# SandraLouise/SVJedi-graph

Hardware: NVIDIA B200
Metric: gaf_alignments_filtered_assigned_per_sec (higher is better)
Workload: dtype u8/int64

## Files before the change

### include/svjg.h

```cpp
#ifndef SVJG_H
#define SVJG_H

#include <stddef.h>
#include <stdint.h>

#ifdef __cplusplus
extern "C" {
#endif

#define SVJG_OK 0
#define SVJG_E_CUDA 1
#define SVJG_E_ARG 2
#define SVJG_E_IO 3
#define SVJG_E_JSON 4
#define SVJG_E_INPUT 5
#define SVJG_E_HITS_OVERFLOW 6
#define SVJG_E_NOMEM 7
#define SVJG_E_UNSUPPORTED 8

#define SVJG_BAD_COLUMNS 1
#define SVJG_BAD_INT 2
#define SVJG_BAD_ALEN 3
#define SVJG_BAD_PATH 4
#define SVJG_BAD_ALTNODE 5
// ... 18 lines not shown
int64_t svjg_tables_alt_node_len(const svjg_tables *t, const char *name, uint32_t len);
uint64_t svjg_tables_image_hash(const svjg_tables *t);
const char *svjg_tables_sv_id(const svjg_tables *t, uint32_t i, uint32_t *len);
uint32_t svjg_tables_find_sv(const svjg_tables *t, const char *sv_id, uint32_t len);
#define SVJG_FLAG_EXACT_CHECKS 1u
#define SVJG_FLAG_FORCE_GENERAL 2u
int svjg_tables_set_flags(svjg_tables *t, uint32_t flags);
int svjg_tables_clone(const svjg_tables *t, svjg_tables **out);
int svjg_tables_to_device(svjg_tables *t, int device);

typedef struct svjg_filter_stats {
    uint64_t n_hits;
    uint64_t n_records;
    uint64_t n_multi;
    uint64_t n_checks;
    uint64_t status;
    uint64_t err_offset;
    uint64_t n_generic;
    uint64_t n_exact;
} svjg_filter_stats;

int svjg_filter_reset(uint32_t *d_counts, uint32_t num_sv, svjg_filter_stats *d_stats, void *stream);
int svjg_filter_device(const svjg_tables *t, const uint8_t *d_gaf, uint64_t n_bytes, uint64_t base_offset,
                       int64_t d_over, uint32_t *d_counts, uint32_t *d_hit_sv2, uint32_t *d_hit_off,
                       uint32_t *d_hit_len, uint64_t hit_cap, svjg_filter_stats *d_stats, void *stream);

uint64_t svjg_translate_newlines(uint8_t *p, uint64_t n);

#define SVJG_TUNE_TILE_BYTES 1
#define SVJG_TUNE_TILE_LINES 2
#define SVJG_TUNE_SCAN_BLOCKS 3
#define SVJG_TUNE_SCAN_ONLY 4
#define SVJG_TUNE_POOL_UNITS 5
int svjg_filter_tune(int knob, int value);
int svjg_filter_profile(int enable);
int svjg_filter_scan_ms(float *ms);

int svjg_filter_host(svjg_tables *t, const uint8_t *gaf, uint64_t n_bytes, int64_t d_over, uint32_t *counts,
                     uint32_t *hit_sv2, uint64_t *hit_off, uint32_t *hit_len, uint64_t hit_cap,
                     svjg_filter_stats *stats);

int svjg_filter_json_host(svjg_tables *t, const uint8_t *gaf, uint64_t n_bytes, int64_t d_over, uint32_t *counts,
                          svjg_filter_stats *stats, const char **json, uint64_t *json_len);
int svjg_filter_json_begin(svjg_tables *t, const uint8_t *gaf, uint64_t n_bytes, int64_t d_over, uint32_t *counts,
                           svjg_filter_stats *stats);
int svjg_filter_json_finish(svjg_tables *t, const char **json, uint64_t *json_len);
int svjg_filter_json_begin_at(svjg_tables *t, const uint8_t *gaf, uint64_t n_bytes, uint64_t base, int64_t d_over,
                              uint32_t *counts, svjg_filter_stats *stats);
int svjg_filter_json_gather(svjg_tables **ts, int n, const uint32_t *counts_sum);
int svjg_filter_json_write(svjg_tables *t, const char *path, uint64_t slice_bytes, uint64_t *json_len);

int svjg_hits_min_identity(const uint8_t *gaf, uint64_t n_bytes, uint32_t *hit_sv2, uint64_t *hit_off, uint32_t *hit_len,
                           uint64_t *n_hits, double min_identity, uint32_t *counts, uint32_t num_sv);

#define SVJG_GT_GENOTYPED 1
#define SVJG_GT_HALVED_0 2
#define SVJG_GT_HALVED_1 4
#define SVJG_GT_NEED_K 8

int svjg_genotype_device(const uint32_t *d_counts, const uint32_t *d_sv_index, const uint8_t *d_svtype,
                         uint32_t n, int64_t min_support, double log10_1me, double log10_e,
                         double log10_half, const double *d_lut, uint32_t lut_nmax,
                         const double *d_k_override, int64_t *d_pl, uint8_t *d_gt, uint32_t *d_ad2,
                         uint8_t *d_flags, void *stream);

int svjg_genotype_host(const uint32_t *counts, uint32_t num_counts, const uint32_t *sv_index, const uint8_t *svtype,
// ... 84 lines not shown
```

### svjedi-graph_b200/csrc/filter.cu

```cuda
#include <cooperative_groups.h>
#include <cuda_runtime.h>

#include <algorithm>
#include <cstdlib>
#include <map>
#include <mutex>

#include "svjg_internal.h"

namespace cg = cooperative_groups;
using namespace svjg;

namespace {

constexpr int TILE_MIN = 1024;
constexpr int TILE_LINES = 30;
constexpr int LOOKAHEAD = 1024;
constexpr int HEAD = 32;
constexpr int WARPS = 4;
constexpr int THREADS = WARPS * 32;
constexpr int SPARE = 32;

template <int MB_, int TILE_MAX_>
struct Geo {
    static constexpr int MB = MB_;
    static constexpr int TILE_MAX = TILE_MAX_;
    static constexpr int WIN = HEAD + TILE_MAX + LOOKAHEAD;
    static constexpr int NLCAP = WIN / 20 + 1;
    static constexpr int BMWORDS = WIN / 32 + 3;
    static constexpr int OFF_NL = WIN + SPARE;
    static constexpr int OFF_TAB = (OFF_NL + 2 * NLCAP + 15) & ~15;
    static constexpr int OFF_XD = OFF_TAB + 4 * BMWORDS;
    static constexpr int OFF_NS = OFF_XD + 4 * BMWORDS;
    static constexpr int OFF_TKO = OFF_NS + 4 * BMWORDS;
    static constexpr int OFF_LREC = (OFF_TKO + 32 + 15) & ~15;
    static constexpr int WARP_SMEM = (OFF_LREC + 32 * 8 + 127) & ~127;
    static constexpr int SMEM = WARP_SMEM * WARPS;
    static_assert(TILE_MAX % 32 == 0 && WIN + SPARE < 65536, "window offsets are 16 bit");
    static_assert((SMEM + 1024 + 64) * MB <= 233472, "MB blocks must fit an SM's 228 KB of shared memory");
};
typedef Geo<6, 4992> Geo6;
typedef Geo<8, 3360> Geo8;

constexpr int FLAT_THREADS = 256;

constexpr uint32_t FLAG_EXACT_CHECKS = SVJG_FLAG_EXACT_CHECKS;
constexpr uint32_t FLAG_FORCE_GENERAL = SVJG_FLAG_FORCE_GENERAL;
constexpr uint32_t FLAG_STOP_AFTER_SCAN = 1u << 8;
constexpr uint32_t COMMA_PATH = 0xFFFFFFFFu;

struct Scratch {
    uint32_t *cnt;
    uint32_t *exact;
    uint4 *slab;
    uint4 *pool;
    uint32_t cap_exact, cap_pool;
};

struct FilterArgs {
    const uint8_t *gaf;
    uint64_t n;
    uint64_t base;
    int64_t d_over;
    DevTables tb;
    uint32_t *counts;
    uint32_t *hit_sv2, *hit_off, *hit_len;
    uint64_t *hit_off64;
    uint64_t hit_cap;
    unsigned long long *stats;
    uint32_t flags;
    uint32_t one;
    Scratch sc;
    uint32_t skip;
    uint32_t tile_max;
    uint32_t tile_lines;
};

struct Local {
    uint32_t n_rec = 0, n_multi = 0, n_generic = 0;
    uint64_t n_checks = 0;
};
// ... 614 lines not shown
    }
    return v;
}

__device__ __forceinline__ uint64_t warp_incl_scan64(uint64_t v, int lane) {
#pragma unroll
    for (int d = 1; d < 32; d <<= 1) {
        uint64_t o = __shfl_up_sync(0xFFFFFFFFu, v, d);
        if (lane >= d) v += o;
    }
    return v;
}

__device__ __forceinline__ uint32_t bm_bits(const uint32_t *bm, uint32_t pos) {
    const uint32_t w = pos >> 5;
    return __funnelshift_r(bm[w], bm[w + 1], pos & 31u);
}
__device__ __forceinline__ uint32_t low_bits(int n) { return __funnelshift_lc(0xFFFFFFFFu, 0u, uint32_t(max(n, 0))); }
__device__ __forceinline__ uint32_t next_tab(const uint32_t *bm, uint32_t pos, uint32_t end) {
    for (uint32_t q = pos; q < end; q += 32) {
        const uint32_t m = bm_bits(bm, q) & low_bits(int(end - q));
        if (m) return q + uint32_t(__ffs(m) - 1);
    }
    return end;
}
__device__ __forceinline__ uint64_t bm64(const uint32_t *bm, uint32_t pos) {
    const uint32_t w = pos >> 5, sh = pos & 31u;
    const uint32_t b0 = bm[w], b1 = bm[w + 1], b2 = bm[w + 2];
    return (uint64_t(__funnelshift_r(b1, b2, sh)) << 32) | __funnelshift_r(b0, b1, sh);
}
__device__ __forceinline__ uint64_t low_bits64(int n) { return (uint64_t(low_bits(n - 32)) << 32) | low_bits(n); }

__device__ __forceinline__ uint32_t dec4(uint32_t w) {
    uint32_t t = w & 0x0F0F0F0Fu;
    t = t * 10u + (t >> 8);
    t &= 0x00FF00FFu;
    return (t * 100u + (t >> 16)) & 0xFFFFu;
}
__device__ __forceinline__ uint32_t clear_low_bytes(uint32_t w, int n) {
    return w & __funnelshift_lc(0u, 0xFFFFFFFFu, uint32_t(max(n, 0)) * 8u);
}
__device__ __forceinline__ bool pnode_find(const DevTables &tb, uint64_t c0, uint64_t c1, uint32_t ka, uint32_t kb,
                                           uint32_t &id, uint32_t &alt_len, uint32_t &roles) {
    uint32_t i = pnode_hash(c0, c1, ka, kb) & tb.pnode_mask;
    for (;;) {
        const uint4 *sp = reinterpret_cast<const uint4 *>(tb.pnodes + i);
        const uint4 lo = __ldg(sp), hi = __ldg(sp + 1);
        if (!hi.z) return false;
        if (lo.x == uint32_t(c0) && lo.y == uint32_t(c0 >> 32) && lo.z == uint32_t(c1) && lo.w == uint32_t(c1 >> 32) &&
            hi.x == ka && hi.y == kb) {
            id = (hi.z & PN_ID_MASK) - 1u;
            roles = hi.z >> 28;
            alt_len = hi.w;
            return true;
        }
        i = (i + 1) & tb.pnode_mask;
    }
}

__device__ __forceinline__ uint32_t link_dirs(uint32_t rolesA, uint32_t sA, uint32_t rolesB, uint32_t sB) {
    const uint32_t fwd = (rolesA >> sA) & (rolesB >> (2u + sB)) & 1u;
    const uint32_t rev = (rolesB >> (sB ^ 1u)) & (rolesA >> (2u + (sA ^ 1u))) & 1u;
    return fwd | (rev << 1);
}

struct SmemBytes {
    const uint8_t *p;
    __device__ __forceinline__ uint32_t u8(uint32_t i) const { return p[i]; }
    __device__ __forceinline__ uint32_t u32(uint32_t al) const { return *reinterpret_cast<const uint32_t *>(p + al); }
};
// ... 168 lines not shown
        bad |= __any_sync(0xFFFFFFFFu, act && !n.plain);
        total += __shfl_sync(0xFFFFFFFFu, warp_incl_scan64(n.nlen, lane), 31);
        from = __shfl_sync(0xFFFFFFFFu, nxt, 31);
    }
    __syncwarp();
    if (bad) return false;
    bool clash = false;
    for (uint32_t c0 = 0; c0 < cnt; c0 += 32) {
        const uint32_t t = c0 + uint32_t(lane);
        const uint32_t mine = t < cnt ? __ldcg(&slab[t].z) : 0u;
        const uint32_t upto = min(c0 + 32u, cnt);
        for (uint32_t j = 0; j < upto; ++j) clash |= j < t && t < cnt && __ldcg(&slab[j].z) == mine;
    }
    if (__any_sync(0xFFFFFFFFu, clash)) return false;
    uint64_t before = 0;
    for (uint32_t c0 = 0; c0 < cnt; c0 += 32) {
        const uint32_t t = c0 + uint32_t(lane);
        const bool act = t < cnt;
        const uint4 me = act ? __ldcg(slab + t) : make_uint4(NO_NODE, 0, 0, 0);
        const uint4 lf = act && t ? __ldcg(slab + t - 1) : make_uint4(NO_NODE, 0, 0, 0);
        const uint64_t incl = warp_incl_scan64(me.y, lane);
        const uint64_t pre = before + incl - me.y;
        const bool ok = (int64_t(pre) - lts >= a.d_over) && (int64_t(total - pre) - ltail >= a.d_over);
        const uint32_t dirs = link_dirs(lf.w >> 1, lf.w & 1u, me.w >> 1, me.w & 1u);
        const bool want = act && t && lf.x != NO_NODE && me.x != NO_NODE && dirs && (ok || (a.flags & FLAG_EXACT_CHECKS));
        probe_links(a, want, lf.x, lf.w & 1u, me.x, me.w & 1u, dirs, ok, off, len, lt_mask, n_checks);
        before += __shfl_sync(0xFFFFFFFFu, incl, 31);
    }
    n_checks = __reduce_add_sync(0xFFFFFFFFu, n_checks);
    if (lane == 0 && n_checks) atomicAdd(a.stats + 3, (unsigned long long)n_checks);
    return true;
}

template <class G>
__global__ void __launch_bounds__(THREADS, G::MB) scan_kernel(const __grid_constant__ FilterArgs a) {
    extern __shared__ __align__(128) uint8_t smem_all[];
    __shared__ __align__(8) uint64_t mbars[WARPS];
    __shared__ uint32_t next_tile[WARPS];

    const int lane = threadIdx.x & 31, warp = threadIdx.x >> 5;
    const uint32_t lt_mask = (1u << lane) - 1u;
    uint8_t *win = smem_all + warp * G::WARP_SMEM;
    uint16_t *nl = reinterpret_cast<uint16_t *>(win + G::OFF_NL);
    uint32_t *tabb = reinterpret_cast<uint32_t *>(win + G::OFF_TAB);
    uint32_t *xdb = reinterpret_cast<uint32_t *>(win + G::OFF_XD);
    uint32_t *nsb = reinterpret_cast<uint32_t *>(win + G::OFF_NS);
    uint8_t *tko = win + G::OFF_TKO;
    uint2 *lrec = reinterpret_cast<uint2 *>(win + G::OFF_LREC);
    uint64_t *mbar = &mbars[warp];
    const SmemBytes src{win};

    if (lane == 0) mbar_init(mbar, 1);
    for (int i = lane; i < G::BMWORDS; i += 32) tabb[i] = 0, xdb[i] = 0, nsb[i] = 0;
    for (int i = G::WIN + lane; i < G::WIN + SPARE; i += 32) win[i] = 0;
    __syncwarp();
    uint32_t phase = 0;
    uint32_t u_rec = 0, u_multi = 0, n_checks = 0;
    const uint32_t one = a.one;
    const uint32_t n_workers = gridDim.x * WARPS;

    cudaGridDependencySynchronize();
    cudaTriggerProgrammaticLaunchCompletion();
    const uint32_t tile_bytes = a.sc.cnt[4];
    const uint32_t n_tiles = uint32_t((a.n + tile_bytes - 1) / tile_bytes);
    const uint32_t win_bytes = HEAD + tile_bytes + LOOKAHEAD, n_pairs = win_bytes / 32u;

    for (uint32_t tile = blockIdx.x * WARPS + warp; tile < n_tiles; tile = next_tile[warp], __syncwarp()) {
        const uint64_t tile_start = uint64_t(tile) * tile_bytes;
        const uint64_t g0 = tile_start ? tile_start - HEAD : 0;
        const uint32_t dst0 = tile_start ? 0 : HEAD;
        uint64_t g1 = tile_start + tile_bytes + LOOKAHEAD;
        if (g1 > a.n) g1 = a.n;
        const bool at_eof = (g1 == a.n);
        const uint32_t nbytes = uint32_t(g1 - g0);
        const uint32_t bulk = nbytes & ~15u;
        const uint32_t valid_end = dst0 + nbytes;
        const uint32_t wbase = uint32_t(tile_start) - HEAD;

        if (lane == 0) {
            if (bulk) {
                asm volatile("fence.proxy.async.shared::cta;" ::: "memory");
// ... 113 lines not shown
                    }
                    plain &= pe < e && pe > ps;
                    const uint32_t n7 = min(pe + 1u, e);
                    uint64_t tt = bm64(tabb, n7);
                    const uint64_t xt = bm64(xdb, n7) & ~tt;
                    plain &= xt != 0;
                    const uint32_t l7 = uint32_t(__ffsll((long long)xt)) - 1u;
                    tt &= low_bits64(int(l7));
                    const uint32_t ntab = uint32_t(__popcll(tt));
                    const bool last_is_tab = l7 != 0 && ((tt >> ((l7 - 1u) & 63u)) & 1ull) != 0;
                    plain &= (ntab == 6 && last_is_tab) || (ntab == 5 && !last_is_tab && n7 + l7 == e);
                    plain &= (tt & ((tt >> 1) | 1ull)) == 0;
                    c6 = pe;
                    c7 = n7 + uint32_t(__ffsll((long long)tt)) - 1u;
                    tt &= tt - 1;
                    c8 = n7 + uint32_t(__ffsll((long long)tt)) - 1u;
                    tt &= tt - 1;
                    c9 = n7 + uint32_t(__ffsll((long long)tt)) - 1u;
                    tt &= tt - 1;
                    const uint32_t p10 = n7 + uint32_t(__ffsll((long long)tt)) - 1u;
                    plain = plain && win[p10 + 1] != '0';
                    if (!plain) {
                        exact = true;
                    } else if (!is_delim(win[ps])) {
                        exact = has_comma(win, ps, pe);
                    } else if (ntok >= 2) {
                        if (a.flags & FLAG_FORCE_GENERAL) exact = true;
                        else want = ntok;
                    }
                }
            }
            __syncwarp();
            int32_t ts = 0, tail = 0;
            if (want) {
                const uint32_t n_tlen = c7 - c6 - 1u, n_ts = c8 - c7 - 1u, n_te = c9 - c8 - 1u;
                if (max(n_tlen, max(n_ts, n_te)) <= 9u) {
                    ts = int32_t(dec9(src, c8, n_ts));
                    tail = int32_t(dec9(src, c7, n_tlen)) - int32_t(dec9(src, c9, n_te)) - 1;
                    lrec[lane] = make_uint2(s | ((e - s + (has_nl ? 1u : 0u)) << 16), ps | (pe << 16));
                } else {
                    exact = true;
                    want = 0;
                }
            }
            __syncwarp();
            uint32_t pend = want > 32u ? 0u : want;
            while (__any_sync(0xFFFFFFFFu, pend != 0)) {
                const uint32_t incl = warp_incl_scan(pend, lane);
                const bool take = pend != 0 && incl <= 32u;
                const uint32_t takeb = __ballot_sync(0xFFFFFFFFu, take);
                const uint32_t ntk = __shfl_sync(0xFFFFFFFFu, incl, 31 - __clz(takeb));
                const uint32_t first = incl - pend;
                const uint32_t startmask = __reduce_or_sync(0xFFFFFFFFu, take ? (1u << first) : 0u);
                if (take) tko[__popc(takeb & lt_mask)] = uint8_t(lane);
                __syncwarp();
                const bool is_tok = uint32_t(lane) < ntk;
                uint32_t own_l = 0, idx = 0;
                if (is_tok) {
                    const uint32_t below = startmask & (0xFFFFFFFFu >> (31 - lane));
                    own_l = tko[__popc(below) - 1];
                    idx = uint32_t(lane) - uint32_t(31 - __clz(below));
                }
                const uint2 lr = lrec[own_l];
                const uint32_t lpath = lr.y;
                const uint32_t lcnt = __shfl_sync(0xFFFFFFFFu, pend, own_l);
                uint32_t tpos = 0;
                if (is_tok) tpos = find_node(nsb, lpath & 0xFFFFu, idx);
                const uint32_t nxt = __shfl_down_sync(0xFFFFFFFFu, tpos, 1);
                Node nd;
                uint32_t plus = 0;
                if (is_tok) {
                    plus = win[tpos - 1u] == '>';
                    nd = resolve_node(src, xdb, a.tb, tpos, idx + 1u < lcnt ? nxt - 1u : lpath >> 16);
                }
                const uint32_t nid = nd.nid, nlen = nd.nlen, akey = nd.akey;
                const uint32_t lfirst = uint32_t(lane) - idx;
                const uint32_t line_lanes = low_bits(int(lcnt)) << lfirst;
                const uint32_t twins = __match_any_sync(0xFFFFFFFFu, akey) & line_lanes;
                bool clash = (twins & ~(1u << lane)) != 0;
                uint64_t lsum = nlen;
#pragma unroll
                for (int d = 1; d < 32; d <<= 1) {
                    const uint64_t o = __shfl_up_sync(0xFFFFFFFFu, lsum, d);
                    if (uint32_t(d) <= idx) lsum += o;
                }
                uint64_t pre_l = lsum - nlen, pre_r = pre_l;
                uint32_t splus = plus, sl = __shfl_up_sync(0xFFFFFFFFu, plus, 1);
                if (__any_sync(0xFFFFFFFFu, is_tok && clash)) {
                    const int twin0 = is_tok ? __ffs(twins) - 1 : lane;
                    const uint32_t f_nid = __shfl_sync(0xFFFFFFFFu, nid, twin0);
                    const uint64_t f_sum = __shfl_sync(0xFFFFFFFFu, lsum, twin0);
                    const uint32_t f_len = __shfl_sync(0xFFFFFFFFu, nlen, twin0);
                    splus = __shfl_sync(0xFFFFFFFFu, plus, twin0);
                    sl = __shfl_up_sync(0xFFFFFFFFu, splus, 1);
                    pre_l = __shfl_up_sync(0xFFFFFFFFu, f_sum, 1);
                    pre_r = f_sum - f_len;
                    clash = clash && !(nid != NO_NODE && f_nid == nid);
                }
                const uint32_t bad = __reduce_or_sync(0xFFFFFFFFu, (is_tok && (!nd.plain || clash)) ? (1u << own_l) : 0u);
                const uint64_t total = __shfl_sync(0xFFFFFFFFu, lsum, is_tok ? lfirst + lcnt - 1u : 0u);
                const uint32_t idl = __shfl_up_sync(0xFFFFFFFFu, nid, 1);
                const int64_t lts = __shfl_sync(0xFFFFFFFFu, ts, own_l), ltail = __shfl_sync(0xFFFFFFFFu, tail, own_l);
                const uint32_t loff = wbase + (lr.x & 0xFFFFu), llen = lr.x >> 16;
                const bool ok = (int64_t(pre_l) - lts >= a.d_over) && (int64_t(total - pre_r) - ltail >= a.d_over);
                const uint32_t dirs = link_dirs(__shfl_up_sync(0xFFFFFFFFu, nd.roles, 1), sl, nd.roles, splus);
                const bool look = is_tok && idx >= 1 && !((bad >> own_l) & 1u) && idl != NO_NODE && nid != NO_NODE && dirs &&
                                  (ok || (a.flags & FLAG_EXACT_CHECKS));
                probe_links(a, look, idl, sl, nid, splus, dirs, ok, loff, llen, lt_mask, n_checks);
                if (take) {
                    if ((bad >> lane) & 1u) exact = true;
                    pend = 0;
                }
                u_multi += __popc(takeb & ~bad);
                __syncwarp();
            }
            for (uint32_t longb = __ballot_sync(0xFFFFFFFFu, want > 32u); longb; longb &= longb - 1) {
                const int L = __ffs(longb) - 1;
                const uint2 lr = lrec[L];
                const bool done = long_line(a, src, nsb, xdb, a.sc.slab + size_t(blockIdx.x * WARPS + warp) * SLAB_N, SLAB_N, lane,
                                            __shfl_sync(0xFFFFFFFFu, want, L), lr.y & 0xFFFFu, lr.y >> 16,
                                            __shfl_sync(0xFFFFFFFFu, ts, L), __shfl_sync(0xFFFFFFFFu, tail, L),
                                            wbase + (lr.x & 0xFFFFu), lr.x >> 16);
                if (!done && lane == L) exact = true;
                u_multi += done;
            }
            const uint32_t xb = __ballot_sync(0xFFFFFFFFu, exact);
            if (xb) {
                uint32_t xbase = 0;
                if (lane == 0) xbase = atomicAdd(a.sc.cnt + 2, uint32_t(__popc(xb)));
                xbase = __shfl_sync(0xFFFFFFFFu, xbase, 0);
                if (exact) {
                    const uint32_t idx = xbase + __popc(xb & lt_mask);
                    if (idx < a.sc.cap_exact) a.sc.exact[idx] = wbase + s;
                    else report(a, SVJG_BAD_SHORTLINE, wbase + s);
                }
            }
        }
        __syncwarp();
    }
    n_checks = __reduce_add_sync(0xFFFFFFFFu, n_checks);
    if (lane == 0) {
        if (u_rec) atomicAdd(a.stats + 1, (unsigned long long)u_rec);
        if (u_multi) atomicAdd(a.stats + 2, (unsigned long long)u_multi);
        if (n_checks) atomicAdd(a.stats + 3, (unsigned long long)n_checks);
    }
}

__device__ __noinline__ bool giant_line(const FilterArgs &a, uint32_t ps, uint32_t pe, uint32_t ntok, int64_t ts, int64_t tail,
                                        uint32_t off, uint32_t len, int lane, Local &loc) {
    if (ps < 64u) return false;
    const uint32_t w0 = (ps >> 5) - 1u, nw = (pe >> 5) - w0 + 4u;
    const uint32_t bm16 = (nw + 3u) / 4u;
    const uint32_t need = 2u * bm16 + ntok;
    uint32_t base = 0;
    if (lane == 0) base = atomicAdd(a.sc.cnt + 5, need);
    base = __shfl_sync(0xFFFFFFFFu, base, 0);
    if (uint64_t(base) + need > a.sc.cap_pool) return false;
    uint32_t *nsb = reinterpret_cast<uint32_t *>(a.sc.pool + base), *xdb = reinterpret_cast<uint32_t *>(a.sc.pool + base + bm16);
    for (uint32_t w = uint32_t(lane); w < nw; w += 32) {
        const uint64_t pos = uint64_t(w0 + w) * 32u;
        uint32_t d = 0, x = 0;
        if (pos + 32 <= a.n) {
            const uint4 v0 = __ldg(reinterpret_cast<const uint4 *>(a.gaf + pos)), v1 = __ldg(reinterpret_cast<const uint4 *>(a.gaf + pos + 16));
            d = mask16(v0, IsDelim{1u}) | (mask16(v1, IsDelim{1u}) << 16);
            x = mask16(v0, IsNonDigit{1u}) | (mask16(v1, IsNonDigit{1u}) << 16);
        } else {
            for (uint32_t k = 0; k < 32; ++k) {
// ... 89 lines not shown
    for (uint64_t k = i; k < n; k += stride) counts[k] = 0;
    if (i < 8) stats[i] = (i == 5) ? ~0ull : 0ull;
}

template <typename... P, typename... A>
cudaError_t launch_pdl(void (*kernel)(P...), unsigned grid, unsigned block, size_t smem, cudaStream_t st, A &&...args) {
    cudaLaunchAttribute attr[1];
    attr[0].id = cudaLaunchAttributeProgrammaticStreamSerialization;
    attr[0].val.programmaticStreamSerializationAllowed = 1;
    cudaLaunchConfig_t cfg = {};
    cfg.gridDim = dim3(grid);
    cfg.blockDim = dim3(block);
    cfg.dynamicSmemBytes = smem;
    cfg.stream = st;
    cfg.attrs = attr;
    cfg.numAttrs = 1;
    return cudaLaunchKernelEx(&cfg, kernel, static_cast<A &&>(args)...);
}

struct DevCfg {
    int sms = 0;
    int grid_cap = 0;
    int min_blocks = 0;
    uint32_t tile_max = 0, tile_lines = 0;
    uint32_t smem = 0;
    cudaEvent_t ev0 = nullptr, ev1 = nullptr;
    bool timed = false;
};
std::mutex g_cfg_mu;
std::map<int, DevCfg> g_cfg;
bool g_profile = false;

struct Knobs {
    int tile_bytes = 0, tile_lines = 0, scan_blocks = 0, scan_only = 0, pool_units = 0;
};
Knobs g_knobs;

template <class G>
int configure_scan(DevCfg &c) {
    c.tile_max = G::TILE_MAX;
    c.tile_lines = g_knobs.tile_lines > 0 ? uint32_t(g_knobs.tile_lines) : uint32_t(TILE_LINES);
    c.smem = G::SMEM;
    c.min_blocks = G::MB;
    SVJG_CUDA(cudaFuncSetAttribute(scan_kernel<G>, cudaFuncAttributeMaxDynamicSharedMemorySize, int(c.smem)));
    int occ = 0;
    SVJG_CUDA(cudaOccupancyMaxActiveBlocksPerMultiprocessor(&occ, scan_kernel<G>, THREADS, c.smem));
    if (occ < 1) return set_error(SVJG_E_CUDA, "scan kernel does not fit on an SM");
    c.grid_cap = c.sms * occ;
    return SVJG_OK;
}

int device_config(DevCfg **out) {
    int dev = 0;
    SVJG_CUDA(cudaGetDevice(&dev));
    std::lock_guard<std::mutex> lock(g_cfg_mu);
    auto it = g_cfg.find(dev);
    if (it == g_cfg.end()) {
        DevCfg c;
        SVJG_CUDA(cudaDeviceGetAttribute(&c.sms, cudaDevAttrMultiProcessorCount, dev));
        const int rc = g_knobs.scan_blocks == 8 ? configure_scan<Geo8>(c) : configure_scan<Geo6>(c);
        if (rc) return rc;
        cudaMemPool_t pool;
        SVJG_CUDA(cudaDeviceGetDefaultMemPool(&pool, dev));
        uint64_t keep = ~0ull;
        SVJG_CUDA(cudaMemPoolSetAttribute(pool, cudaMemPoolAttrReleaseThreshold, &keep));
        SVJG_CUDA(cudaEventCreate(&c.ev0));
        SVJG_CUDA(cudaEventCreate(&c.ev1));
        it = g_cfg.emplace(dev, c).first;
    }
    *out = &it->second;
    return SVJG_OK;
}

}

extern "C" int svjg_filter_reset(uint32_t *d_counts, uint32_t num_sv, svjg_filter_stats *d_stats, void *stream) {
    if (!d_counts || !d_stats) return set_error(SVJG_E_ARG, "svjg_filter_reset: NULL argument");
    uint64_t n = uint64_t(num_sv) * 2;
    int blocks = int(std::min<uint64_t>(1184, (n + 255) / 256));
    if (blocks < 1) blocks = 1;
    reset_kernel<<<blocks, 256, 0, (cudaStream_t)stream>>>(d_counts, n, reinterpret_cast<unsigned long long *>(d_stats));
    SVJG_CUDA(cudaGetLastError());
    return SVJG_OK;
}

extern "C" int svjg_filter_device(const svjg_tables *t, const uint8_t *d_gaf, uint64_t n_bytes, uint64_t base_offset,
                                  int64_t d_over, uint32_t *d_counts, uint32_t *d_hit_sv2, uint32_t *d_hit_off,
                                  uint32_t *d_hit_len, uint64_t hit_cap, svjg_filter_stats *d_stats, void *stream) {
    return svjg::filter_device_abs(t, d_gaf, n_bytes, base_offset, d_over, d_counts, d_hit_sv2, d_hit_off, nullptr, d_hit_len,
                                   hit_cap, d_stats, stream);
}

extern "C" int svjg_filter_tune(int knob, int value) {
    if (value < 0) return set_error(SVJG_E_ARG, "svjg_filter_tune: negative value");
    std::lock_guard<std::mutex> lock(g_cfg_mu);
    switch (knob) {
        case SVJG_TUNE_TILE_BYTES: g_knobs.tile_bytes = value; break;
        case SVJG_TUNE_SCAN_ONLY: g_knobs.scan_only = value; break;
        case SVJG_TUNE_POOL_UNITS: g_knobs.pool_units = value; break;
        case SVJG_TUNE_TILE_LINES:
        case SVJG_TUNE_SCAN_BLOCKS:
            if (knob == SVJG_TUNE_TILE_LINES) g_knobs.tile_lines = value;
            else g_knobs.scan_blocks = value;
            for (auto &kv : g_cfg) {
                cudaEventDestroy(kv.second.ev0);
                cudaEventDestroy(kv.second.ev1);
            }
            g_cfg.clear();
            break;
        default: return set_error(SVJG_E_ARG, "svjg_filter_tune: unknown knob");
    }
    return SVJG_OK;
}
extern "C" int svjg_filter_profile(int enable) {
    g_profile = enable != 0;
    return SVJG_OK;
}
extern "C" int svjg_filter_scan_ms(float *ms) {
    if (!ms) return set_error(SVJG_E_ARG, "svjg_filter_scan_ms: NULL argument");
    DevCfg *c = nullptr;
    if (int rc = device_config(&c)) return rc;
    if (!c->timed) return set_error(SVJG_E_ARG, "svjg_filter_scan_ms: no profiled call on this device");
    SVJG_CUDA(cudaEventSynchronize(c->ev1));
    SVJG_CUDA(cudaEventElapsedTime(ms, c->ev0, c->ev1));
    return SVJG_OK;
}

int svjg::filter_device_abs(const svjg_tables *t, const uint8_t *d_gaf, uint64_t n_bytes, uint64_t base_offset, int64_t d_over,
                            uint32_t *d_counts, uint32_t *d_hit_sv2, uint32_t *d_hit_off, uint64_t *d_hit_off64,
                            uint32_t *d_hit_len, uint64_t hit_cap, svjg_filter_stats *d_stats, void *stream, bool inside_buffer) {
    if (!t || t->device < 0) return set_error(SVJG_E_ARG, "svjg_filter_device: tables are not on a device");
    uint32_t skip = 0;
// ... 2 lines not shown
        if (base_offset < skip) return set_error(SVJG_E_ARG, "svjg_filter_device: shard inside a buffer without the bytes in front of it");
        d_gaf -= skip;
        n_bytes += n_bytes ? skip : 0;
        base_offset -= skip;
    }
    if (!d_counts || !d_stats || (n_bytes && !d_gaf)) return set_error(SVJG_E_ARG, "svjg_filter_device: NULL argument");
    if (hit_cap && (!d_hit_sv2 || (!d_hit_off && !d_hit_off64) || !d_hit_len))
        return set_error(SVJG_E_ARG, "svjg_filter_device: NULL hit buffer");
    if (reinterpret_cast<uintptr_t>(d_gaf) & 15) return set_error(SVJG_E_ARG, "svjg_filter_device: d_gaf must be 16-byte aligned");
    if (n_bytes >= 0xFFFF0000ull) return set_error(SVJG_E_ARG, "svjg_filter_device: shard must be smaller than 4 GiB");
    if (n_bytes == 0) return SVJG_OK;
    cudaStream_t st = (cudaStream_t)stream;
    DevCfg *cfg = nullptr;
    if (int rc = device_config(&cfg)) return rc;
    FilterArgs a;
    a.gaf = d_gaf;
    a.n = n_bytes;
    a.base = base_offset;
    a.d_over = d_over;
    a.tb = t->dev;
    a.counts = d_counts;
    a.hit_sv2 = d_hit_sv2;
    a.hit_off = d_hit_off;
    a.hit_off64 = d_hit_off64;
    a.hit_len = d_hit_len;
    a.hit_cap = hit_cap;
    a.stats = reinterpret_cast<unsigned long long *>(d_stats);
    a.flags = t->filter_flags;
    a.one = 1;
    a.skip = skip;
    a.tile_max = cfg->tile_max;
    a.tile_lines = cfg->tile_lines;
    if (g_knobs.scan_only) a.flags |= FLAG_STOP_AFTER_SCAN;
    if (g_knobs.tile_bytes) a.flags |= uint32_t(std::min(65535, g_knobs.tile_bytes)) << 16;

    Scratch &sc = a.sc;
    sc.cap_exact = uint32_t(n_bytes / 16 + 64);
    sc.cap_pool = uint32_t(std::min<uint64_t>(4u << 20, std::max<uint64_t>(64u << 10, n_bytes / 256)));
    if (g_knobs.pool_units) sc.cap_pool = uint32_t(g_knobs.pool_units);
    auto up = [](size_t x) { return (x + 255) & ~size_t(255); };
    const size_t o_cnt = 0, o_ex = up(64), o_slab = o_ex + up(size_t(sc.cap_exact) * 4),
                 o_pool = o_slab + up(size_t(cfg->grid_cap) * WARPS * SLAB_N * sizeof(uint4)),
                 total = o_pool + up(size_t(sc.cap_pool) * sizeof(uint4));
    uint8_t *ws = nullptr;
    SVJG_CUDA(cudaMallocAsync(reinterpret_cast<void **>(&ws), total, st));
    sc.cnt = reinterpret_cast<uint32_t *>(ws + o_cnt);
    sc.exact = reinterpret_cast<uint32_t *>(ws + o_ex);
    sc.slab = reinterpret_cast<uint4 *>(ws + o_slab);
    sc.pool = reinterpret_cast<uint4 *>(ws + o_pool);

    const uint32_t max_tiles = uint32_t((n_bytes + TILE_MIN - 1) / TILE_MIN);
    const int scan_grid = int(std::min<uint32_t>((max_tiles + WARPS - 1) / WARPS, uint32_t(cfg->grid_cap)));
    probe_kernel<<<1, PROBE_THREADS, 0, st>>>(a);
    cudaError_t le = cudaGetLastError();
    if (g_profile) cudaEventRecord(cfg->ev0, st);
    if (le == cudaSuccess)
        le = launch_pdl(cfg->min_blocks == 8 ? scan_kernel<Geo8> : scan_kernel<Geo6>, scan_grid, THREADS, cfg->smem, st, a);
    if (g_profile) cudaEventRecord(cfg->ev1, st), cfg->timed = true;
    if (le == cudaSuccess && !(a.flags & FLAG_STOP_AFTER_SCAN))
        le = launch_pdl(exact_kernel, cfg->sms * 2, FLAT_THREADS, 0, st, a);
    if (le == cudaSuccess) le = cudaGetLastError();
    cudaError_t fe = cudaFreeAsync(ws, st);
    SVJG_CUDA(le);
    SVJG_CUDA(fe);
    return SVJG_OK;
}
```

### svjedi-graph_b200/svjg/capi.py

```python
from __future__ import annotations

import ctypes as C
import os

_HERE = os.path.dirname(os.path.abspath(__file__))
LIB_PATH = os.path.join(os.path.dirname(_HERE), "lib", "libsvjg.so")

OK, E_CUDA, E_ARG, E_IO, E_JSON, E_INPUT, E_HITS_OVERFLOW, E_NOMEM, E_UNSUPPORTED = range(9)
GT_GENOTYPED, GT_HALVED_0, GT_HALVED_1, GT_NEED_K = 1, 2, 4, 8
NO_SV = 0xFFFFFFFF
FLAG_EXACT_CHECKS, FLAG_FORCE_GENERAL = 1, 2
TUNE_TILE_BYTES, TUNE_TILE_LINES, TUNE_SCAN_BLOCKS, TUNE_SCAN_ONLY, TUNE_POOL_UNITS = 1, 2, 3, 4, 5

BAD_REASONS = {
    1: "blank line or fewer than 12 columns",
    2: "non-integer numeric column",
    3: "Alen == 0 without an id:f: tag",
    4: "empty or malformed path column",
    5: "alt node missing from the GFA",
    6: "reference-node name without start-end coordinates",
    7: "svs_edges entry without ':' in the sv id or with a bad allele",
    8: "line shorter than 16 bytes",
    9: "integer with more than 18 digits",
}


class SvjgError(RuntimeError):
    def __init__(self, code, message):
        super().__init__(f"libsvjg error {code}: {message}")
        self.code = code


class FilterStats(C.Structure):
    _fields_ = [(n, C.c_uint64) for n in
                ("n_hits", "n_records", "n_multi", "n_checks", "status", "err_offset", "n_generic", "n_exact")]

    def as_dict(self):
        return {n: int(getattr(self, n)) for n, _ in self._fields_}


def _load():
    if not os.path.exists(LIB_PATH):
        raise ImportError(
            f"{LIB_PATH} not found: build it with `python -c 'import __graft_entry__ as g; g.build()'` "
            "(or `make -C svjedi-graph_b200/csrc`). There is no CPU fallback.")
# ... 103 lines not shown
```

Before: 8.064 billion.

## Pack per-line round records in shared memory and narrow path-length prefix sums

Each round's line record now carries offset, length, node count, ts and tail in one 16-byte shared-memory slot written by the taking lane. This replaces the token-owner byte table plus several warp shuffles for ts/tail/count. The prefix sum over node lengths runs in 32-bit unless some node is very long, avoiding 64-bit shuffles in the common case. dec4 uses dp4a, and a stop-after-lines profiling knob with a phase-split script is added; window offsets shrink to 13 bits, which tightens the static window limit.

```diff
diff --git a/include/svjg.h b/include/svjg.h
--- a/include/svjg.h
+++ b/include/svjg.h
@@ -74,6 +74,7 @@
 #define SVJG_TUNE_SCAN_BLOCKS 3
 #define SVJG_TUNE_SCAN_ONLY 4
 #define SVJG_TUNE_POOL_UNITS 5
+#define SVJG_TUNE_STOP_AFTER_LINES 6
 int svjg_filter_tune(int knob, int value);
 int svjg_filter_profile(int enable);
 int svjg_filter_scan_ms(float *ms);
diff --git a/profiles/phase_split.py b/profiles/phase_split.py
--- /dev/null
+++ b/profiles/phase_split.py
@@ -0,0 +1,158 @@
+#!/usr/bin/env python3
+import argparse
+import ctypes as C
+import json
+import os
+import statistics
+import subprocess
+import sys
+
+ROOT = os.path.dirname(os.path.dirname(os.path.abspath(__file__)))
+for p in (ROOT, os.path.join(ROOT, "svjedi-graph_b200")):
+    if p not in sys.path:
+        sys.path.insert(0, p)
+
+TILE_MAX, TILE_LINES, TILE_MIN, HEAD, PROBE_BYTES = 4992, 30, 1024, 32, 64 << 10
+
+
+def tile_bytes(gaf):
+    n16 = min(len(gaf), PROBE_BYTES) // 16
+    total = gaf[:n16 * 16].count(b"\n")
+    tile = TILE_MAX
+    if total:
+        tile = min(n16 * 16 * TILE_LINES // total, TILE_MAX) & ~31
+        slack = min(n16 * 24 // total, 512)
+        steps = (HEAD + tile + slack) // 1024
+        if steps >= 2:
+            tile = (steps * 1024 - HEAD - slack) & ~31
+    return max(TILE_MIN, min(tile, TILE_MAX))
+
+
+def path_nodes(line):
+    cols = line.split(b"\t", 6)
+    if len(cols) < 7 or not cols[5] or cols[5][0] not in b"<>":
+        return None
+    return sum(1 for piece in cols[5].replace(b">", b"<").split(b"<") if piece)
+
+
+def rounds_of(gaf, tb):
+    n_rounds = n_lines = n_nodes = n_long = 0
+    tile, pend = -1, []
+
+    def flush(lines):
+        nonlocal n_rounds, n_lines, n_nodes
+        for k0 in range(0, len(lines), 32):
+            todo = [c for c in lines[k0:k0 + 32] if c]
+            while todo:
+                s, i = 0, 0
+                while i < len(todo) and s + todo[i] <= 32:
+                    s += todo[i]
+                    i += 1
+                n_rounds += 1
+                n_lines += i
+                n_nodes += s
+                todo = todo[i:]
+
+    off = 0
+    for line in gaf.split(b"\n"):
+        t = off // tb
+        if t != tile:
+            flush(pend)
+            tile, pend = t, []
+        n = path_nodes(line) if line else None
+        c = 0
+        if n is not None and n >= 2:
+            if n <= 32:
+                c = n
+            else:
+                n_long += 1
+        pend.append(c)
+        off += len(line) + 1
+    flush(pend)
+    return n_rounds, n_lines, n_nodes, n_long
+
+
+def gpu_info():
+    try:
+        out = subprocess.run(["nvidia-smi", "--query-gpu=name,power.limit,clocks.sm,clocks.max.sm", "--format=csv,noheader"],
+                             capture_output=True, text=True, timeout=30).stdout.strip().splitlines()
+        return out[0] if out else None
+    except (OSError, subprocess.SubprocessError):
+        return None
+
+
+def main():
+    ap = argparse.ArgumentParser()
+    ap.add_argument("--workloads", default="C2,C3,C4,C5")
+    ap.add_argument("--catalogue", default="full", choices=["scaled", "full"])
+    ap.add_argument("--scale", type=float, default=0.01)
+    ap.add_argument("--iters", type=int, default=10, help="profiled calls per mode and rep")
+    ap.add_argument("--reps", type=int, default=5)
+    args = ap.parse_args()
+
+    import torch
+
+    import bench
+    from svjg import alnfilter, capi
+
+    if not torch.cuda.is_available():
+        raise SystemExit("phase_split.py needs a GPU")
+    lib = capi.lib
+    modes = {"whole": None, "lines": capi.TUNE_STOP_AFTER_LINES, "bytes": capi.TUNE_SCAN_ONLY}
+    info = gpu_info()
+    for wl in args.workloads.split(","):
+        ns = argparse.Namespace(workload=wl, scale=args.scale, catalogue=args.catalogue)
+        g, vcf, gaf, gfa_text, scale, _ = bench.workload(ns, 0)
+        tables = alnfilter.Tables.from_memory(g.edges_json(), gfa_text).to_device(0)
+        gaf_bytes = gaf.encode()
+        d_gaf = torch.frombuffer(bytearray(gaf_bytes), dtype=torch.uint8).cuda()
+        filt = alnfilter.DeviceFilter(tables, hit_cap=1024, device=0)
+        filt.reset()
+        filt.run(d_gaf)
+        filt = alnfilter.DeviceFilter(tables, hit_cap=filt.read_stats()["n_hits"] + 1024, device=0)
+        sp = C.c_void_p(torch.cuda.current_stream().cuda_stream)
+
+        def timed(knob, n):
+            if knob:
+                capi.check(lib.svjg_filter_tune(knob, 1))
+            capi.check(lib.svjg_filter_profile(1))
+            tot, ms = 0.0, C.c_float()
+            try:
+                for _ in range(n):
+                    capi.check(lib.svjg_filter_reset(filt.counts.data_ptr(), tables.num_sv, filt.stats.data_ptr(), sp))
+                    capi.check(lib.svjg_filter_device(tables._h, d_gaf.data_ptr(), len(gaf_bytes), 0, 100, filt.counts.data_ptr(),
+                                                      filt.hit_sv2.data_ptr(), filt.hit_off.data_ptr(), filt.hit_len.data_ptr(),
+                                                      filt.hit_cap, filt.stats.data_ptr(), sp))
+                    capi.check(lib.svjg_filter_scan_ms(C.byref(ms)))
+                    tot += ms.value
+            finally:
+                capi.check(lib.svjg_filter_profile(0))
+                if knob:
+                    capi.check(lib.svjg_filter_tune(knob, 0))
+            return tot / n
+
+        for knob in modes.values():
+            timed(knob, 3)
+        samples = {m: [] for m in modes}
+        for _ in range(args.reps):
+            for m, knob in modes.items():
+                samples[m].append(timed(knob, args.iters))
+        ms = {m: statistics.median(v) for m, v in samples.items()}
+        tb = tile_bytes(gaf_bytes)
+        n_rounds, n_lines, n_nodes, n_long = rounds_of(gaf_bytes, tb)
+        print(json.dumps({
+            "workload": f"{wl} x{scale:g} catalogue {args.catalogue}", "gpu": info, "n_bytes": len(gaf_bytes),
+            "n_records": gaf_bytes.count(b"\n"), "tile_bytes": tb, "tiles": -(-len(gaf_bytes) // tb),
+            "rounds": n_rounds, "round_lines": n_lines, "round_nodes": n_nodes,
+            "nodes_per_round": round(n_nodes / max(1, n_rounds), 2), "lines_per_round": round(n_lines / max(1, n_rounds), 2),
+            "long_lines": n_long,
+            "scan_ms": {m: round(v, 5) for m, v in ms.items()},
+            "rounds_ms": round(ms["whole"] - ms["lines"], 5), "line_phase_ms": round(ms["lines"] - ms["bytes"], 5),
+            "ns_per_round": round((ms["whole"] - ms["lines"]) * 1e6 / max(1, n_rounds), 3),
+            "spread_ms": {m: round(max(v) - min(v), 5) for m, v in samples.items()},
+        }), flush=True)
+        del filt, tables, d_gaf
+
+
+if __name__ == "__main__":
+    main()
diff --git a/svjedi-graph_b200/csrc/filter.cu b/svjedi-graph_b200/csrc/filter.cu
--- a/svjedi-graph_b200/csrc/filter.cu
+++ b/svjedi-graph_b200/csrc/filter.cu
@@ -32,11 +32,10 @@
     static constexpr int OFF_TAB = (OFF_NL + 2 * NLCAP + 15) & ~15;
     static constexpr int OFF_XD = OFF_TAB + 4 * BMWORDS;
     static constexpr int OFF_NS = OFF_XD + 4 * BMWORDS;
-    static constexpr int OFF_TKO = OFF_NS + 4 * BMWORDS;
-    static constexpr int OFF_LREC = (OFF_TKO + 32 + 15) & ~15;
-    static constexpr int WARP_SMEM = (OFF_LREC + 32 * 8 + 127) & ~127;
+    static constexpr int OFF_LREC = (OFF_NS + 4 * BMWORDS + 15) & ~15;
+    static constexpr int WARP_SMEM = (OFF_LREC + 16 * 16 + 127) & ~127;
     static constexpr int SMEM = WARP_SMEM * WARPS;
-    static_assert(TILE_MAX % 32 == 0 && WIN + SPARE < 65536, "window offsets are 16 bit");
+    static_assert(TILE_MAX % 32 == 0 && WIN + SPARE <= 8192, "window offsets are 13 bit (a round's line records)");
     static_assert((SMEM + 1024 + 64) * MB <= 233472, "MB blocks must fit an SM's 228 KB of shared memory");
 };
 typedef Geo<6, 4992> Geo6;
@@ -47,6 +46,7 @@
 constexpr uint32_t FLAG_EXACT_CHECKS = SVJG_FLAG_EXACT_CHECKS;
 constexpr uint32_t FLAG_FORCE_GENERAL = SVJG_FLAG_FORCE_GENERAL;
 constexpr uint32_t FLAG_STOP_AFTER_SCAN = 1u << 8;
+constexpr uint32_t FLAG_STOP_AFTER_LINES = 1u << 9;
 constexpr uint32_t COMMA_PATH = 0xFFFFFFFFu;
 
 struct Scratch {
@@ -727,10 +727,8 @@
 __device__ __forceinline__ uint64_t low_bits64(int n) { return (uint64_t(low_bits(n - 32)) << 32) | low_bits(n); }
 
 __device__ __forceinline__ uint32_t dec4(uint32_t w) {
-    uint32_t t = w & 0x0F0F0F0Fu;
-    t = t * 10u + (t >> 8);
-    t &= 0x00FF00FFu;
-    return (t * 100u + (t >> 16)) & 0xFFFFu;
+    const uint32_t t = w & 0x0F0F0F0Fu;
+    return __dp4a(t, 0x0000010Au, 0u) * 100u + __dp4a(t, 0x010A0000u, 0u);
 }
 __device__ __forceinline__ uint32_t clear_low_bytes(uint32_t w, int n) {
     return w & __funnelshift_lc(0u, 0xFFFFFFFFu, uint32_t(max(n, 0)) * 8u);
@@ -965,6 +963,35 @@
     return true;
 }
 
+template <class T>
+__device__ __forceinline__ bool round_verdicts(const Node &nd, uint32_t plus, uint32_t idx, bool is_tok, uint32_t twins,
+                                               bool any_clash, uint32_t tlast, int32_t lts, int32_t ltail, int64_t d_over,
+                                               uint32_t &splus, uint32_t &sl, bool &clash) {
+    const int lane = threadIdx.x & 31;
+    T lsum = nd.nlen;
+#pragma unroll
+    for (int d = 1; d < 32; d <<= 1) {
+        const T o = __shfl_up_sync(0xFFFFFFFFu, lsum, d);
+        if (uint32_t(d) <= idx) lsum += o;
+    }
+    T pre_l = lsum - nd.nlen, pre_r = pre_l;
+    splus = plus;
+    sl = __shfl_up_sync(0xFFFFFFFFu, plus, 1);
+    if (any_clash) {
+        const int twin0 = is_tok ? __ffs(twins) - 1 : lane;
+        const uint32_t f_nid = __shfl_sync(0xFFFFFFFFu, nd.nid, twin0);
+        const T f_sum = __shfl_sync(0xFFFFFFFFu, lsum, twin0);
+        const uint32_t f_len = __shfl_sync(0xFFFFFFFFu, nd.nlen, twin0);
+        splus = __shfl_sync(0xFFFFFFFFu, plus, twin0);
+        sl = __shfl_up_sync(0xFFFFFFFFu, splus, 1);
+        pre_l = __shfl_up_sync(0xFFFFFFFFu, f_sum, 1);
+        pre_r = f_sum - f_len;
+        clash = clash && !(nd.nid != NO_NODE && f_nid == nd.nid);
+    }
+    const T total = __shfl_sync(0xFFFFFFFFu, lsum, tlast);
+    return (int64_t(pre_l) - lts >= d_over) && (int64_t(total - pre_r) - ltail >= d_over);
+}
+
 template <class G>
 __global__ void __launch_bounds__(THREADS, G::MB) scan_kernel(const __grid_constant__ FilterArgs a) {
     extern __shared__ __align__(128) uint8_t smem_all[];
@@ -978,8 +1005,7 @@
     uint32_t *tabb = reinterpret_cast<uint32_t *>(win + G::OFF_TAB);
     uint32_t *xdb = reinterpret_cast<uint32_t *>(win + G::OFF_XD);
     uint32_t *nsb = reinterpret_cast<uint32_t *>(win + G::OFF_NS);
-    uint8_t *tko = win + G::OFF_TKO;
-    uint2 *lrec = reinterpret_cast<uint2 *>(win + G::OFF_LREC);
+    uint4 *lrec = reinterpret_cast<uint4 *>(win + G::OFF_LREC);
     uint64_t *mbar = &mbars[warp];
     const SmemBytes src{win};
 
@@ -1159,18 +1185,20 @@
             }
             __syncwarp();
             int32_t ts = 0, tail = 0;
+            uint32_t rx = s, ry = 0;
             if (want) {
                 const uint32_t n_tlen = c7 - c6 - 1u, n_ts = c8 - c7 - 1u, n_te = c9 - c8 - 1u;
                 if (max(n_tlen, max(n_ts, n_te)) <= 9u) {
                     ts = int32_t(dec9(src, c8, n_ts));
                     tail = int32_t(dec9(src, c7, n_tlen)) - int32_t(dec9(src, c9, n_te)) - 1;
-                    lrec[lane] = make_uint2(s | ((e - s + (has_nl ? 1u : 0u)) << 16), ps | (pe << 16));
+                    rx |= ((e - s + (has_nl ? 1u : 0u)) << 13) | (min(want, 63u) << 26);
+                    ry = ps | (pe << 16);
                 } else {
                     exact = true;
                     want = 0;
                 }
             }
-            __syncwarp();
+            if (a.flags & FLAG_STOP_AFTER_LINES) want = 0;
             uint32_t pend = want > 32u ? 0u : want;
             while (__any_sync(0xFFFFFFFFu, pend != 0)) {
                 const uint32_t incl = warp_incl_scan(pend, lane);
@@ -1179,75 +1207,58 @@
                 const uint32_t ntk = __shfl_sync(0xFFFFFFFFu, incl, 31 - __clz(takeb));
                 const uint32_t first = incl - pend;
                 const uint32_t startmask = __reduce_or_sync(0xFFFFFFFFu, take ? (1u << first) : 0u);
-                if (take) tko[__popc(takeb & lt_mask)] = uint8_t(lane);
+                if (take) lrec[__popc(takeb & lt_mask)] = make_uint4(rx, ry, uint32_t(ts), uint32_t(tail));
                 __syncwarp();
                 const bool is_tok = uint32_t(lane) < ntk;
-                uint32_t own_l = 0, idx = 0;
+                uint32_t ord = 0, idx = 0;
                 if (is_tok) {
                     const uint32_t below = startmask & (0xFFFFFFFFu >> (31 - lane));
-                    own_l = tko[__popc(below) - 1];
+                    ord = __popc(below) - 1;
                     idx = uint32_t(lane) - uint32_t(31 - __clz(below));
                 }
-                const uint2 lr = lrec[own_l];
-                const uint32_t lpath = lr.y;
-                const uint32_t lcnt = __shfl_sync(0xFFFFFFFFu, pend, own_l);
+                const uint4 lr = lrec[ord];
+                const uint32_t lcnt = lr.x >> 26;
                 uint32_t tpos = 0;
-                if (is_tok) tpos = find_node(nsb, lpath & 0xFFFFu, idx);
+                if (is_tok) tpos = find_node(nsb, lr.y & 0xFFFFu, idx);
                 const uint32_t nxt = __shfl_down_sync(0xFFFFFFFFu, tpos, 1);
                 Node nd;
                 uint32_t plus = 0;
                 if (is_tok) {
                     plus = win[tpos - 1u] == '>';
-                    nd = resolve_node(src, xdb, a.tb, tpos, idx + 1u < lcnt ? nxt - 1u : lpath >> 16);
-                }
-                const uint32_t nid = nd.nid, nlen = nd.nlen, akey = nd.akey;
+                    nd = resolve_node(src, xdb, a.tb, tpos, idx + 1u < lcnt ? nxt - 1u : lr.y >> 16);
+                }
                 const uint32_t lfirst = uint32_t(lane) - idx;
-                const uint32_t line_lanes = low_bits(int(lcnt)) << lfirst;
-                const uint32_t twins = __match_any_sync(0xFFFFFFFFu, akey) & line_lanes;
+                const uint32_t twins = __match_any_sync(0xFFFFFFFFu, nd.akey) & (low_bits(int(lcnt)) << lfirst);
                 bool clash = (twins & ~(1u << lane)) != 0;
-                uint64_t lsum = nlen;
-#pragma unroll
-                for (int d = 1; d < 32; d <<= 1) {
-                    const uint64_t o = __shfl_up_sync(0xFFFFFFFFu, lsum, d);
-                    if (uint32_t(d) <= idx) lsum += o;
-                }
-                uint64_t pre_l = lsum - nlen, pre_r = pre_l;
-                uint32_t splus = plus, sl = __shfl_up_sync(0xFFFFFFFFu, plus, 1);
-                if (__any_sync(0xFFFFFFFFu, is_tok && clash)) {
-                    const int twin0 = is_tok ? __ffs(twins) - 1 : lane;
-                    const uint32_t f_nid = __shfl_sync(0xFFFFFFFFu, nid, twin0);
-                    const uint64_t f_sum = __shfl_sync(0xFFFFFFFFu, lsum, twin0);
-                    const uint32_t f_len = __shfl_sync(0xFFFFFFFFu, nlen, twin0);
-                    splus = __shfl_sync(0xFFFFFFFFu, plus, twin0);
-                    sl = __shfl_up_sync(0xFFFFFFFFu, splus, 1);
-                    pre_l = __shfl_up_sync(0xFFFFFFFFu, f_sum, 1);
-                    pre_r = f_sum - f_len;
-                    clash = clash && !(nid != NO_NODE && f_nid == nid);
-                }
-                const uint32_t bad = __reduce_or_sync(0xFFFFFFFFu, (is_tok && (!nd.plain || clash)) ? (1u << own_l) : 0u);
-                const uint64_t total = __shfl_sync(0xFFFFFFFFu, lsum, is_tok ? lfirst + lcnt - 1u : 0u);
-                const uint32_t idl = __shfl_up_sync(0xFFFFFFFFu, nid, 1);
-                const int64_t lts = __shfl_sync(0xFFFFFFFFu, ts, own_l), ltail = __shfl_sync(0xFFFFFFFFu, tail, own_l);
-                const uint32_t loff = wbase + (lr.x & 0xFFFFu), llen = lr.x >> 16;
-                const bool ok = (int64_t(pre_l) - lts >= a.d_over) && (int64_t(total - pre_r) - ltail >= a.d_over);
+                const bool any_clash = __any_sync(0xFFFFFFFFu, is_tok && clash);
+                const uint32_t tlast = is_tok ? lfirst + lcnt - 1u : 0u;
+                uint32_t splus = plus, sl;
+                const bool ok = __any_sync(0xFFFFFFFFu, nd.nlen >= (1u << 27))
+                                    ? round_verdicts<uint64_t>(nd, plus, idx, is_tok, twins, any_clash, tlast, int32_t(lr.z),
+                                                               int32_t(lr.w), a.d_over, splus, sl, clash)
+                                    : round_verdicts<uint32_t>(nd, plus, idx, is_tok, twins, any_clash, tlast, int32_t(lr.z),
+                                                               int32_t(lr.w), a.d_over, splus, sl, clash);
+                const uint32_t bad = __reduce_or_sync(0xFFFFFFFFu, (is_tok && (!nd.plain || clash)) ? (1u << ord) : 0u);
+                const uint32_t idl = __shfl_up_sync(0xFFFFFFFFu, nd.nid, 1);
+                const uint32_t loff = wbase + (lr.x & 0x1FFFu), llen = (lr.x >> 13) & 0x1FFFu;
                 const uint32_t dirs = link_dirs(__shfl_up_sync(0xFFFFFFFFu, nd.roles, 1), sl, nd.roles, splus);
-                const bool look = is_tok && idx >= 1 && !((bad >> own_l) & 1u) && idl != NO_NODE && nid != NO_NODE && dirs &&
+                const bool look = is_tok && idx >= 1 && !((bad >> ord) & 1u) && idl != NO_NODE && nd.nid != NO_NODE && dirs &&
                                   (ok || (a.flags & FLAG_EXACT_CHECKS));
-                probe_links(a, look, idl, sl, nid, splus, dirs, ok, loff, llen, lt_mask, n_checks);
+                probe_links(a, look, idl, sl, nd.nid, splus, dirs, ok, loff, llen, lt_mask, n_checks);
                 if (take) {
-                    if ((bad >> lane) & 1u) exact = true;
+                    if ((bad >> __popc(takeb & lt_mask)) & 1u) exact = true;
                     pend = 0;
                 }
-                u_multi += __popc(takeb & ~bad);
+                u_multi += __popc(takeb) - __popc(bad);
                 __syncwarp();
             }
             for (uint32_t longb = __ballot_sync(0xFFFFFFFFu, want > 32u); longb; longb &= longb - 1) {
                 const int L = __ffs(longb) - 1;
-                const uint2 lr = lrec[L];
+                const uint32_t lx = __shfl_sync(0xFFFFFFFFu, rx, L), ly = __shfl_sync(0xFFFFFFFFu, ry, L);
                 const bool done = long_line(a, src, nsb, xdb, a.sc.slab + size_t(blockIdx.x * WARPS + warp) * SLAB_N, SLAB_N, lane,
-                                            __shfl_sync(0xFFFFFFFFu, want, L), lr.y & 0xFFFFu, lr.y >> 16,
+                                            __shfl_sync(0xFFFFFFFFu, want, L), ly & 0xFFFFu, ly >> 16,
                                             __shfl_sync(0xFFFFFFFFu, ts, L), __shfl_sync(0xFFFFFFFFu, tail, L),
-                                            wbase + (lr.x & 0xFFFFu), lr.x >> 16);
+                                            wbase + (lx & 0x1FFFu), (lx >> 13) & 0x1FFFu);
                 if (!done && lane == L) exact = true;
                 u_multi += done;
             }
@@ -1258,8 +1269,9 @@
                 xbase = __shfl_sync(0xFFFFFFFFu, xbase, 0);
                 if (exact) {
                     const uint32_t idx = xbase + __popc(xb & lt_mask);
-                    if (idx < a.sc.cap_exact) a.sc.exact[idx] = wbase + s;
-                    else report(a, SVJG_BAD_SHORTLINE, wbase + s);
+                    const uint32_t off = wbase + (rx & 0x1FFFu);
+                    if (idx < a.sc.cap_exact) a.sc.exact[idx] = off;
+                    else report(a, SVJG_BAD_SHORTLINE, off);
                 }
             }
         }
@@ -1415,7 +1427,7 @@
 bool g_profile = false;
 
 struct Knobs {
-    int tile_bytes = 0, tile_lines = 0, scan_blocks = 0, scan_only = 0, pool_units = 0;
+    int tile_bytes = 0, tile_lines = 0, scan_blocks = 0, scan_only = 0, pool_units = 0, stop_after_lines = 0;
 };
 Knobs g_knobs;
 
@@ -1481,6 +1493,7 @@
         case SVJG_TUNE_TILE_BYTES: g_knobs.tile_bytes = value; break;
         case SVJG_TUNE_SCAN_ONLY: g_knobs.scan_only = value; break;
         case SVJG_TUNE_POOL_UNITS: g_knobs.pool_units = value; break;
+        case SVJG_TUNE_STOP_AFTER_LINES: g_knobs.stop_after_lines = value; break;
         case SVJG_TUNE_TILE_LINES:
         case SVJG_TUNE_SCAN_BLOCKS:
             if (knob == SVJG_TUNE_TILE_LINES) g_knobs.tile_lines = value;
@@ -1549,6 +1562,7 @@
     a.tile_max = cfg->tile_max;
     a.tile_lines = cfg->tile_lines;
     if (g_knobs.scan_only) a.flags |= FLAG_STOP_AFTER_SCAN;
+    if (g_knobs.stop_after_lines) a.flags |= FLAG_STOP_AFTER_LINES;
     if (g_knobs.tile_bytes) a.flags |= uint32_t(std::min(65535, g_knobs.tile_bytes)) << 16;
 
     Scratch &sc = a.sc;
@@ -1574,7 +1588,7 @@
     if (le == cudaSuccess)
         le = launch_pdl(cfg->min_blocks == 8 ? scan_kernel<Geo8> : scan_kernel<Geo6>, scan_grid, THREADS, cfg->smem, st, a);
     if (g_profile) cudaEventRecord(cfg->ev1, st), cfg->timed = true;
-    if (le == cudaSuccess && !(a.flags & FLAG_STOP_AFTER_SCAN))
+    if (le == cudaSuccess && !(a.flags & (FLAG_STOP_AFTER_SCAN | FLAG_STOP_AFTER_LINES)))
         le = launch_pdl(exact_kernel, cfg->sms * 2, FLAT_THREADS, 0, st, a);
     if (le == cudaSuccess) le = cudaGetLastError();
     cudaError_t fe = cudaFreeAsync(ws, st);
diff --git a/svjedi-graph_b200/svjg/capi.py b/svjedi-graph_b200/svjg/capi.py
--- a/svjedi-graph_b200/svjg/capi.py
+++ b/svjedi-graph_b200/svjg/capi.py
@@ -10,7 +10,7 @@
 GT_GENOTYPED, GT_HALVED_0, GT_HALVED_1, GT_NEED_K = 1, 2, 4, 8
 NO_SV = 0xFFFFFFFF
 FLAG_EXACT_CHECKS, FLAG_FORCE_GENERAL = 1, 2
-TUNE_TILE_BYTES, TUNE_TILE_LINES, TUNE_SCAN_BLOCKS, TUNE_SCAN_ONLY, TUNE_POOL_UNITS = 1, 2, 3, 4, 5
+TUNE_TILE_BYTES, TUNE_TILE_LINES, TUNE_SCAN_BLOCKS, TUNE_SCAN_ONLY, TUNE_POOL_UNITS, TUNE_STOP_AFTER_LINES = 1, 2, 3, 4, 5, 6
 
 BAD_REASONS = {
     1: "blank line or fewer than 12 columns",
```

Result: no change. 8.135 billion (median of 6 runs) (+0.9%).
